# NeRdTheNed/deft4j

Measured on AMD Instinct MI355X. Metric: input MB/s on raw-deflate optimise (mode NONE), higher is better.
Workload: dtype u8

## Files before the change

deft4j_amd/csrc/d4g_fused.h:

```cpp
#pragma once
#include "d4g_ops.h"

#define D4F_MAXSLOTS 576
#define D4F_MAXOPS 640
#define D4F_MAXM 256
#define D4F_MAXC 96
#define D4F_MAXH 384
#define D4F_PASSN 1024
#define D4F_LEASTN 64
#define D4F_HDRN 256
#define D4F_SWEEP_K 8
#define D4F_CODE_FIXED 1
#define D4F_MAXROUNDS 16
#define D4F_HS_SLOTS 8
#define D4F_TREE_SLOTS 4

struct D4FCode {
    uint8_t lens[D4G_NLIT + D4G_NDIST];
    int32_t nLit, nDist, type, err;
    int32_t pad[12];
};
struct D4FPairs {
    uint16_t pairs[D4G_MAXPAIRS];
    int32_t nPairs, pad[3];
};
struct D4FHdr {
    uint8_t clLen[32];
    uint32_t flags[10];
    int32_t nCl, bits, base, pad;
    int32_t pad2[2];
};
struct D4FGlob {
    uint32_t* hist;
    D4FCode* code;
    D4FPairs* pairs;
    D4FHdr* hdr;
    int32_t* binBase;
};
#define D4F_GLOB_BYTES ((size_t)D4F_MAXM * D4G_HIST * 4 + (size_t)D4F_MAXC * sizeof(D4FCode) + (size_t)(D4F_MAXC + 1) * sizeof(D4FPairs) + \
                        (size_t)D4F_MAXH * sizeof(D4FHdr) + (size_t)D4F_MAXC * 64 * 4)

struct D4FParams {
    const D4GOp* ops[2];
    int32_t nOps[2];
    int32_t maxRounds;
    int32_t regWords;
    uint32_t caps;
    int32_t pad;
    D4GRoundResult* results;
    int32_t* roundInfo;
    long long* stats;
};
#define D4F_CL_MAXT 48
#define D4F_CL_SLOTS 96
#define D4F_CL_CHUNK (64 * D4F_NWR)
#define D4F_CL_SWEEP_WORDS 16
enum { D4F_CMD_SWEEP = 1, D4F_CMD_APPLY = 2, D4F_CMD_LEAST_WALK = 3, D4F_CMD_LEAST_EXPAND = 4 };
struct D4FClTask {
    int32_t m, code, prune, leaf, mNew, mode, rem, via;
    uint32_t full;
    int32_t pad0[3];
    int32_t cnt, saved;
    unsigned long long h1, h2;
    int32_t bin[3][32];
    int32_t delta[D4G_HIST];
    int32_t pad1[14];
};
static_assert(sizeof(D4FClTask) % 128 == 0, "tasks on cache lines of their own");
struct D4FClCmd {
    int32_t cmd, nItems, nTasks, nk, nChunks, pad0[3];
    int32_t codes[D4F_SWEEP_K];
    int32_t next, done, pad1[14];
    uint32_t neq[D4F_SWEEP_K];
    int32_t pad2[24];
    D4FClTask task[D4F_CL_MAXT];
};
struct D4FClArena {
    int32_t epoch;
    int32_t pad[31];
    D4FClCmd slot[D4F_CL_SLOTS];
};

#define D4F_CAPS(masks, codes, hdrs) ((uint32_t)(masks) | (uint32_t)(hdrs) << 10 | (uint32_t)(codes) << 20)
#define D4F_INFO_FALLBACK 0x10000
#define D4F_INFO_MORE 0x20000

struct D4FSlot { int16_t m, c, h; uint8_t valid, type; int32_t lazy; long long litlen; };
struct D4FPassE { uint32_t key; int32_t saved; int16_t mOut; uint8_t st, pad; };
struct D4FLeastE { uint32_t key; int32_t delta; int16_t mOut; uint8_t st, pad; };
struct D4FHdrE { uint32_t key; int16_t hOut; uint8_t st, pad; };

enum { D4F_Q_SWEEP = 0, D4F_Q_APPLY, D4F_Q_BINBASE, D4F_Q_LEAST, D4F_Q_TREE, D4F_Q_HDR, D4F_Q_HS, D4F_Q_FIXDOT, D4F_NQ };
#define D4F_QCAP_SWEEP D4F_MAXC
#define D4F_QCAP_APPLY 256
#define D4F_QCAP_BINBASE D4F_MAXC
#define D4F_QCAP_LEAST 64
#define D4F_QCAP_TREE 64
#define D4F_QCAP_HDR 256
#define D4F_QCAP_HS D4F_MAXC
#define D4F_QCAP_FIXDOT 4
#define D4F_QTOTAL (D4F_QCAP_SWEEP + D4F_QCAP_APPLY + D4F_QCAP_BINBASE + D4F_QCAP_LEAST + D4F_QCAP_TREE + D4F_QCAP_HDR + D4F_QCAP_HS + D4F_QCAP_FIXDOT)
D4G_DEV int d4f_qcap(int q) {
    return q == D4F_Q_SWEEP ? D4F_QCAP_SWEEP : q == D4F_Q_APPLY ? D4F_QCAP_APPLY : q == D4F_Q_BINBASE ? D4F_QCAP_BINBASE : q == D4F_Q_LEAST ? D4F_QCAP_LEAST
         : q == D4F_Q_TREE ? D4F_QCAP_TREE : q == D4F_Q_HDR ? D4F_QCAP_HDR : q == D4F_Q_HS ? D4F_QCAP_HS : D4F_QCAP_FIXDOT;
}
D4G_DEV int d4f_qoff(int q) {
    int o = 0;
    if (q > D4F_Q_SWEEP) o += D4F_QCAP_SWEEP;
    if (q > D4F_Q_APPLY) o += D4F_QCAP_APPLY;
    if (q > D4F_Q_BINBASE) o += D4F_QCAP_BINBASE;
    if (q > D4F_Q_LEAST) o += D4F_QCAP_LEAST;
    if (q > D4F_Q_TREE) o += D4F_QCAP_TREE;
    if (q > D4F_Q_HDR) o += D4F_QCAP_HDR;
    if (q > D4F_Q_HS) o += D4F_QCAP_HS;
    return o;
}
enum { D4F_H_OPT = 1, D4F_H_POST = 2, D4F_H_PRUNE = 3 };

typedef TreeMem<uint64_t, uint16_t, D4G_NLIT, 16, true> D4FLitTree;
typedef TreeMem<uint64_t, uint16_t, D4G_NDIST, 16, true> D4FDistTree;
struct D4FTreeScr {
    alignas(16) unsigned char tree[(D4FLitTree::bytes(1) + 15) & ~15];
    alignas(16) unsigned char treeD[(D4FDistTree::bytes(1) + 15) & ~15];
    uint32_t hist[D4G_HIST];
    alignas(16) uint8_t lens[D4G_NLIT + D4G_NDIST];
    uint16_t pairs[D4G_MAXPAIRS];
    uint8_t clLen[32];
    uint32_t clFreq[20];
    int32_t nLit, nDist, nCl, nPairs, hdrBits, err, m, pad;
    long long litlen;
};
struct D4FWaveScr {
    uint32_t hist[D4G_HIST];
    uint16_t lc[256];
    uint8_t cl[64];
    uint32_t queue[128];
    int32_t binSize[32], binFreq[32], binZ[32];
    int32_t delta[D4G_HIST];
    int32_t misc[16];
};
struct D4FHdrScr {
    uint16_t pairs[D4G_MAXPAIRS];
    uint8_t clLen[32];
    uint32_t clFreq[20];
    alignas(16) unsigned char tree[256];
    int32_t nCl, nPairs, bits, pad;
};
struct D4FSweepScr {
    uint16_t lc[D4F_SWEEP_K][256];
    uint8_t cl[D4F_SWEEP_K][64];
    uint32_t neq[D4F_SWEEP_K];
    unsigned long long stage[8][D4F_SWEEP_K][2][16];
};
struct D4FHsScr {
    D4GHdrLds H;
    alignas(16) uint8_t comb[D4G_NLIT + D4G_NDIST];
};
union D4FScratch {
    D4FTreeScr tree[D4F_TREE_SLOTS];
    D4FWaveScr wave[8];
    D4FSweepScr sweep;
    D4GLds levelLds;
};
static_assert(sizeof(D4FHdrScr) <= sizeof(D4FWaveScr), "header scratch overlays the wave scratch");

struct D4FLds {
    D4FSlot slot[D4F_MAXSLOTS];
    uint8_t slotReady[D4F_MAXSLOTS];
    uint8_t opStage[D4F_MAXOPS];
    uint16_t opReq[D4F_MAXOPS];
    long long treeLit[D4F_MAXM];
    uint8_t treeC[D4F_MAXM];
    alignas(4) uint8_t treeSt[D4F_MAXM];
    int32_t hdrBits[D4F_MAXH];
    unsigned long long maskH1[D4F_MAXM], maskH2[D4F_MAXM];
    int32_t maskPop[D4F_MAXM];
    uint32_t maskFull[D4F_MAXM];
    alignas(4) uint16_t maskHash[512];
    uint16_t maskStep[D4F_MAXM];
    uint16_t maskHH[D4F_MAXM];
    int32_t treeCand[2][D4F_QCAP_TREE];
    int16_t defHdr[D4F_MAXC];
    uint16_t qAll[D4F_QTOTAL];
    int32_t qn[D4F_NQ];
    int32_t nMask, nHdr, nDone, fallback, progress[2], fixdotSt, fixdotM, step, pad0;
    long long fixdotLit;
    long long red[32];
    int32_t misc[32];
    alignas(16) D4FLeastE least[D4F_LEASTN];
    D4FHdrE hdrReq[D4F_HDRN];
    D4FPassE pass[D4F_PASSN];
    D4FScratch scr;
    unsigned long long codeH[D4F_MAXC];
    alignas(4) uint8_t codeHash[256];
    alignas(4) uint8_t eState[D4F_MAXC];
    alignas(4) uint8_t eEq[D4F_MAXC];
    alignas(4) uint8_t bbState[D4F_MAXC];
    alignas(4) uint8_t hsState[D4F_MAXC];
    int32_t hsBits[D4F_MAXC];
    alignas(4) uint8_t hsLane[D4F_MAXC];
    int32_t nCode, capC;
    D4GCtx c;
    D4GBlock b;
    D4FGlob G;
    const D4GOp* ops;
    int32_t nOps, curType, rounds, info, improved, regWords;
    struct D4FClArena* cl;
    int32_t clEpoch, clDoneWg;
    int32_t which;
    int16_t capM, capH;
    long long curSize;
};

static_assert(sizeof(D4FLds) <= 80 * 1024, "two workgroups per CU: 80 KiB of LDS each");
static_assert(offsetof(D4FLds, codeH) - offsetof(D4FLds, least) >= D4F_HS_SLOTS * sizeof(D4FHsScr), "header-search scratch overlay");
__shared__ D4FLds d4fLds;
#define D4F_TASK __device__ __attribute__((noinline))
// ... 1140 lines not shown
        if (lane < 32) dst.clLen[lane] = H.clLen[lane];
        if (lane < 10) {
            uint32_t fl = 0;
            for (int j = 0; j < 32; j++) { const int i = lane * 32 + j; if (i < nPairs && (H.pairs[i] & D4G_PAIR_EXPANDED)) fl |= 1u << j; }
            dst.flags[lane] = fl;
        }
        if (lane == 0) { dst.nCl = H.nCl; dst.bits = H.bits; dst.base = src.base; F.hdrBits[hNew] = H.bits; }
    }
    d4g_wave_sync();
    if (lane == 0) { e.hOut = (int16_t)hNew; d4g_fence_block(); e.st = 2; }
}

D4F_TASK void d4f_tree_lit(int slotIdx, int m) {
    D4FLds& F = d4fLds;
    D4F_CTX;
    D4FTreeScr& T = F.scr.tree[slotIdx];
    const int lane = threadIdx.x & 63;
    for (int i = lane; i < D4G_NLIT; i += 64) T.hist[i] = G.hist[(size_t)m * D4G_HIST + i];
    for (int i = lane; i < D4G_NLIT / 4; i += 64) ((uint32_t*)T.lens)[i] = 0;
    d4g_wave_sync();
    int ml = 0;
    for (int i = lane; i < 286; i += 64) if (T.hist[i]) ml = i + 1 > ml ? i + 1 : ml;
    const int lastLit = wave_max_i32(ml);
    D4FLitTree tm;
    tm.carve(T.tree, 1);
    const int err = d4f_wave_tree<(D4G_NLIT + 63) / 64>(tm, lastLit, 15, [&](int i) { return T.hist[i]; }, [&](int v, int len) { T.lens[v] = (uint8_t)len; });
    if (lane == 0) { T.nLit = lastLit; T.err = err; T.m = m; }
    d4g_wave_sync();
}
D4F_TASK void d4f_tree_dist(int slotIdx, int m) {
    D4FLds& F = d4fLds;
    D4F_CTX;
    D4FTreeScr& T = F.scr.tree[slotIdx];
    const int lane = threadIdx.x & 63;
    if (lane < D4G_NDIST) { T.hist[D4G_NLIT + lane] = G.hist[(size_t)m * D4G_HIST + D4G_NLIT + lane]; T.lens[D4G_NLIT + lane] = 0; }
    d4g_wave_sync();
    int md = 0;
    if (lane < 30 && T.hist[D4G_NLIT + lane]) md = lane + 1;
    const int lastDist = wave_max_i32(md);
    const bool used = lane < lastDist && T.hist[D4G_NLIT + lane] != 0;
    const int nz = __popcll(d4g_ballot(used));
    int nDist, err = 0;
    if (lastDist == 0) nDist = 1;
    else if (nz <= 1) { nDist = lastDist; if (lane == 0) T.lens[D4G_NLIT + lastDist - 1] = 1; }
    else {
        D4FDistTree tm;
        tm.carve(T.treeD, 1);
        err = d4f_wave_tree<1>(tm, lastDist, 15, [&](int i) { return T.hist[D4G_NLIT + i]; }, [&](int v, int len) { T.lens[D4G_NLIT + v] = (uint8_t)len; });
        nDist = lastDist;
    }
    if (lane == 0) { T.nDist = nDist; T.pad = err; }
    d4g_wave_sync();
}
D4F_TASK void d4f_tree_header(int slotIdx) {
    D4FLds& F = d4fLds;
    D4FTreeScr& T = F.scr.tree[slotIdx];
    const int lane = threadIdx.x & 63;
    long long v = 0;
    for (int i = lane; i < D4G_HIST; i += 64) {
        const unsigned h = T.hist[i];
        if (h) {
            if (i < D4G_NLIT) v += (long long)h * (T.lens[i] + (i >= 257 ? d4g_lsym_ebits(i) : 0));
            else v += (long long)h * (T.lens[i] + d4g_dsym_ebits(i - D4G_NLIT));
        }
    }
    v = wave_sum_i64(v);
    int nPairs, nCl, bits;
    const int err = d4f_wave_default_header(T.lens, T.nLit, T.nDist, T.pairs, T.clFreq, T.clLen, T.tree, nPairs, nCl, bits);
    if (lane == 0) { T.nCl = nCl; T.nPairs = nPairs; T.hdrBits = bits; T.err |= err | T.pad; T.litlen = v; }
    d4g_wave_sync();
}
D4F_TASK void d4f_tree_publish(int slotIdx) {
    D4FLds& F = d4fLds;
    D4F_CTX;
    D4FTreeScr& T = F.scr.tree[slotIdx];
    const int lane = threadIdx.x & 63;
    unsigned long long h = 0;
    const uint32_t* lw = (const uint32_t*)T.lens;
    for (int i = lane; i < (D4G_NLIT + D4G_NDIST) / 4; i += 64) h += d4f_mix1(i, lw[i]);
    h = (unsigned long long)wave_sum_i64((long long)h) + (unsigned long long)T.nLit * 0x100000001b3ULL + ((unsigned long long)T.nDist << 48);
    if (h == 0) h = 1;
    int found = -1;
    uint32_t k = (uint32_t)(h >> 40) & 255u;
    for (int probe = 0; probe < 256; probe++, k = (k + 1) & 255u) {
        const int e = F.codeHash[k];
        if (e == 0) break;
        const int id = e - 1;
        if (F.codeH[id] == h) {
            const D4FCode& cd = G.code[id];
            int bad = 0;
            for (int i = lane; i < (D4G_NLIT + D4G_NDIST) / 4; i += 64) bad |= ((const uint32_t*)cd.lens)[i] != lw[i];
            if (lane == 0) bad |= cd.nLit != T.nLit || cd.nDist != T.nDist || cd.type != D4G_DYNAMIC;
            if (!d4g_ballot(bad)) { found = id; break; }
        }
    }
    int code = found;
    const int nCodeNow = __shfl(F.nCode, 0);
    if (code < 0) {
        code = nCodeNow;
        if (code >= F.capC) { if (lane == 0) F.fallback = 1; code = 0; }
        else {
            D4FCode& cd = G.code[code];
            for (int i = lane; i < (D4G_NLIT + D4G_NDIST) / 4; i += 64) ((uint32_t*)cd.lens)[i] = lw[i];
            if (lane == 0) {
                cd.nLit = T.nLit; cd.nDist = T.nDist; cd.type = D4G_DYNAMIC; cd.err = T.err;
                F.nCode = code + 1;
                F.codeH[code] = h;
                F.defHdr[code] = -1;
                F.eState[code] = 0; F.eEq[code] = 0; F.bbState[code] = 0; F.hsState[code] = 0;
                F.codeHash[k] = (uint8_t)(code + 1);
            }
        }
    }
    d4g_wave_sync();
    if (T.err && lane == 0) atomicAdd(c.errors, 1);
    const int defNow = __shfl((int)F.defHdr[code], 0);
    const int nHdrNow = __shfl(F.nHdr, 0);
    if (defNow < 0) {
        int hid = nHdrNow;
        if (hid >= F.capH) { if (lane == 0) F.fallback = 1; hid = 0; }
        else {
            D4FPairs& pb = G.pairs[1 + code];
            for (int i = lane; i < T.nPairs; i += 64) pb.pairs[i] = T.pairs[i];
            D4FHdr& hd = G.hdr[hid];
            if (lane < 32) hd.clLen[lane] = lane < 19 ? T.clLen[lane] : 0;
            if (lane < 10) hd.flags[lane] = 0;
            if (lane == 0) {
                pb.nPairs = T.nPairs;
                hd.nCl = T.nCl; hd.bits = T.hdrBits; hd.base = 1 + code;
                F.hdrBits[hid] = T.hdrBits;
                F.nHdr = hid + 1;
                F.defHdr[code] = (int16_t)hid;
            }
        }
    }
    d4g_wave_sync();
    if (lane == 0) { F.treeC[T.m] = (uint8_t)code; F.treeLit[T.m] = T.litlen; d4g_fence_block(); F.treeSt[T.m] = 2; }
    d4g_wave_sync();
}

D4F_TASK int d4f_hs_task(int slotIdx, int code) {
    D4FLds& F = d4fLds;
    D4F_CTX;
    D4FHsScr& X = ((D4FHsScr*)&F.least)[slotIdx];
    const int lane = threadIdx.x & 63;
    D4GHdrLds& H = X.H;
    uint8_t* comb = X.comb;
    const D4FCode& cd = G.code[code];
    const int nLit = cd.nLit, n = nLit + cd.nDist;
    for (int i = lane; i < (D4G_NLIT + D4G_NDIST) / 4; i += 64) ((uint32_t*)H.lens)[i] = ((const uint32_t*)cd.lens)[i];
    d4g_wave_sync();
    for (int i = lane; i < D4G_NLIT + D4G_NDIST; i += 64) comb[i] = i >= n ? 0 : i < nLit ? H.lens[i] : H.lens[D4G_NLIT + i - nLit];
    if (lane < 20) H.baseFreq[lane] = 0;
    d4g_wave_sync();
    {
        constexpr int NCH = (D4G_NLIT + D4G_NDIST) / 64;
        unsigned long long sm[NCH];
        int v[NCH];
#pragma unroll
        for (int ch = 0; ch < NCH; ch++) {
            int i = ch * 64 + lane;
            v[ch] = i < n ? (int)comb[i] : -1;
            int pv = (i > 0 && i < n) ? (int)comb[i - 1] : -2;
            sm[ch] = d4g_ballot(i < n && v[ch] != pv);
        }
        int ncx = 0;
#pragma unroll
        for (int ch = 0; ch < NCH; ch++) {
            int i = ch * 64 + lane;
            bool start = (sm[ch] >> lane) & 1;
            int run = 0;
            if (start) {
                int nx = -1;
                unsigned long long m = lane == 63 ? 0ULL : (sm[ch] >> (lane + 1));
                if (m) nx = i + __ffsll((long long)m);
#pragma unroll
                for (int c2 = ch + 1; c2 < NCH; c2++)
                    if (nx < 0 && sm[c2]) nx = c2 * 64 + __ffsll((long long)sm[c2]) - 1;
                if (nx < 0) nx = n;
                run = nx - i;
            }
            bool simple = start && (v[ch] != 0 ? run <= 3 : run <= 2);
            bool cx = start && !simple;
            if (simple) atomicAdd(&H.baseFreq[v[ch]], (unsigned)run);
            unsigned long long cm = d4g_ballot(cx);
// ... 379 lines not shown
    D4FGlob G;
    uint8_t* p = (uint8_t*)state_ptr(c, blk, 1);
    G.hist = (uint32_t*)p; p += (size_t)D4F_MAXM * D4G_HIST * 4;
    G.code = (D4FCode*)p; p += (size_t)D4F_MAXC * sizeof(D4FCode);
    G.pairs = (D4FPairs*)p; p += (size_t)(D4F_MAXC + 1) * sizeof(D4FPairs);
    G.hdr = (D4FHdr*)p; p += (size_t)D4F_MAXH * sizeof(D4FHdr);
    G.binBase = (int32_t*)p;
    return G;
}

__device__ __forceinline__ void d4f_assemble(const D4FGlob& G, D4GState* S, int mid, int cid, int hid, int type, long long litlen) {
    const D4FCode& cd = G.code[cid];
    __syncthreads();
    for (int i = threadIdx.x; i < (D4G_NLIT + D4G_NDIST) / 4; i += blockDim.x) ((uint32_t*)S->litLen)[i] = ((const uint32_t*)cd.lens)[i];
    for (int i = threadIdx.x; i < D4G_HIST; i += blockDim.x) S->hist[i] = G.hist[(size_t)mid * D4G_HIST + i];
    for (int i = threadIdx.x; i < 8; i += blockDim.x) ((uint32_t*)S->clLen)[i] = 0;
    if (type == D4G_DYNAMIC) {
        const D4FHdr& hd = G.hdr[hid];
        const D4FPairs& pb = G.pairs[hd.base];
        const int np = pb.nPairs;
        for (int i = threadIdx.x; i < np; i += blockDim.x) S->pairs[i] = (uint16_t)(pb.pairs[i] | (((hd.flags[i >> 5] >> (i & 31)) & 1u) ? D4G_PAIR_EXPANDED : 0u));
        __syncthreads();
        if (threadIdx.x < 32) S->clLen[threadIdx.x] = hd.clLen[threadIdx.x];
        if (threadIdx.x == 0) { S->nCl = hd.nCl; S->nPairs = np; S->hdrBits = hd.bits; S->nLit = cd.nLit; S->nDist = cd.nDist; }
    } else {
        if (threadIdx.x == 0) { S->nCl = 0; S->nPairs = 0; S->hdrBits = 0; S->nLit = 0; S->nDist = 0; }
    }
    __syncthreads();
    if (threadIdx.x == 0) {
        S->valid = 1; S->type = type; S->maskSlot = 0; S->flags = 0; S->pad0 = 0;
        S->litlenBits = litlen;
        S->sizeBits = litlen + S->hdrBits;
    }
    __syncthreads();
}

D4F_TASK bool d4f_round_setup(const D4GOp* ops0, const D4GOp* ops1, int nOps0, int nOps1) {
    D4FLds& F = d4fLds;
    D4F_CTX;
    const int lane = threadIdx.x & 63, wave = threadIdx.x >> 6;
    const D4GState* cur = state_ptr(c, c.active[d4fLds.which], 0);
    __syncthreads();
    const int curType = cur->type;
    const int prog = curType == D4G_FIXED ? 1 : 0;
    const int nOps = prog ? nOps1 : nOps0;
    for (int i = threadIdx.x; i < (int)(offsetof(D4FLds, scr) / 4); i += blockDim.x) ((uint32_t*)&F)[i] = 0;
    __syncthreads();
    if (threadIdx.x == 0) { F.ops = prog ? ops1 : ops0; F.nOps = nOps; F.curType = curType; F.curSize = cur->sizeBits; }
    if (nOps > D4F_MAXOPS || c.slotsPerBlock > D4F_MAXSLOTS) { __syncthreads(); return false; }
    if (F.nCode > D4F_MAXC - 32) {
        __syncthreads();
        for (int i = threadIdx.x; i < D4F_MAXC; i += blockDim.x) { F.eState[i] = 0; F.eEq[i] = 0; F.bbState[i] = 0; F.hsState[i] = 0; }
        for (int i = threadIdx.x; i < 256; i += blockDim.x) F.codeHash[i] = 0;
        if (threadIdx.x == 0) F.nCode = 2;
        __syncthreads();
    }
    for (int i = threadIdx.x; i < D4F_MAXC; i += blockDim.x) F.defHdr[i] = -1;
    D4FCode& c1 = G.code[D4F_CODE_FIXED];
    for (int i = threadIdx.x; i < D4G_NLIT + D4G_NDIST; i += blockDim.x)
        c1.lens[i] = (uint8_t)(i < 144 ? 8 : i < 256 ? 9 : i < 280 ? 7 : i < 286 ? 8 : i < D4G_NLIT ? 0 : i < D4G_NLIT + 30 ? 5 : 0);
    for (int i = threadIdx.x; i < D4G_HIST; i += blockDim.x) G.hist[i] = cur->hist[i];
    D4FPairs& p0 = G.pairs[0];
    D4FHdr& h0 = G.hdr[0];
    const int np = curType == D4G_DYNAMIC ? cur->nPairs : 0;
    for (int i = threadIdx.x; i < np; i += blockDim.x) p0.pairs[i] = (uint16_t)(cur->pairs[i] & ~D4G_PAIR_EXPANDED);
    if (threadIdx.x < 10) {
        uint32_t fl = 0;
        for (int j = 0; j < 32; j++) { const int i = threadIdx.x * 32 + j; if (i < np && (cur->pairs[i] & D4G_PAIR_EXPANDED)) fl |= 1u << j; }
        h0.flags[threadIdx.x] = fl;
    }
    if (threadIdx.x < 32) h0.clLen[threadIdx.x] = curType == D4G_DYNAMIC ? cur->clLen[threadIdx.x] : 0;
    int pc = 0;
    const uint64_t* m0 = d4f_mask(c, b, 0);
    for (int w = threadIdx.x; w < (int)b.maskWords; w += blockDim.x) pc += __popcll(m0[w]);
    const long long pop = wg_sum_i64(pc, F.red);
    {
        const uint64_t* bmask = c.binMask + b.binMask;
        const int nWords = (int)b.maskWords;
        unsigned nf = 0;
        if (nWords > 4096) nf = (1u << D4G_NBINS) - 1;
        else for (int i = threadIdx.x; i < D4G_NBINS * nWords; i += blockDim.x) {
            const int bin = i / nWords, w = i - bin * nWords;
            if (bmask[(long long)bin * nWords + w] & ~m0[w]) nf |= 1u << bin;
        }
        if (nf) atomicOr((unsigned*)&F.misc[1], nf);
        __syncthreads();
        if (threadIdx.x == 0) F.maskFull[0] = ~(unsigned)F.misc[1] & ((1u << D4G_NBINS) - 1);
    }
    if (wave == 0) {
        const uint32_t* cw = (const uint32_t*)cur->litLen;
        const uint32_t w0 = cw[lane], w1 = lane < 16 ? cw[64 + lane] : 0u;
        const int nLit0 = cur->nLit, nDist0 = cur->nDist;
        unsigned long long h = d4f_mix1(lane, w0) + (lane < 16 ? d4f_mix1(64 + lane, w1) : 0ull);
        h = (unsigned long long)wave_sum_i64((long long)h) + (unsigned long long)nLit0 * 0x100000001b3ULL + ((unsigned long long)nDist0 << 48) +
            (curType == D4G_DYNAMIC ? 0ull : 0x9e3779b97f4a7c15ULL);
        if (h == 0) h = 1;
        int found = -1;
        uint32_t k = (uint32_t)(h >> 40) & 255u;
        for (int probe = 0; probe < 256; probe++, k = (k + 1) & 255u) {
            const int e = F.codeHash[k];
            if (e == 0) break;
            const int id = e - 1;
            if (F.codeH[id] == h) {
                const D4FCode& cd = G.code[id];
                int bad = ((const uint32_t*)cd.lens)[lane] != w0;
                if (lane < 16) bad |= ((const uint32_t*)cd.lens)[64 + lane] != w1;
                if (lane == 0) bad |= cd.nLit != nLit0 || cd.nDist != nDist0 || cd.type != curType;
                if (!d4g_ballot(bad)) { found = id; break; }
            }
        }
        const int nCodeNow = __shfl(F.nCode, 0);
        int code = found;
        if (code < 0) {
            code = nCodeNow;
            D4FCode& cd = G.code[code];
            ((uint32_t*)cd.lens)[lane] = w0;
            if (lane < 16) ((uint32_t*)cd.lens)[64 + lane] = w1;
            if (lane == 0) {
                cd.nLit = nLit0; cd.nDist = nDist0; cd.type = curType; cd.err = 0;
                F.nCode = code + 1;
                F.codeH[code] = h;
                F.codeHash[k] = (uint8_t)(code + 1);
                F.eState[code] = 0; F.eEq[code] = 0; F.bbState[code] = 0; F.hsState[code] = 0;
            }
        }
        if (lane == 0) F.misc[2] = code;
    }
    if (wave == 1 || blockDim.x == 64) {
        const uint16_t hh = d4f_hist_hash(cur->hist);
        if (lane == 0) F.maskHH[0] = hh;
    }
    __syncthreads();
    if (threadIdx.x == 0) {
        c1.nLit = 0; c1.nDist = 0; c1.type = D4G_FIXED; c1.err = 0;
        p0.nPairs = np;
        h0.nCl = cur->nCl; h0.bits = (int32_t)cur->hdrBits; h0.base = 0;
        F.hdrBits[0] = curType == D4G_DYNAMIC ? (int32_t)cur->hdrBits : 0;
        F.nMask = 1; F.nHdr = 1; F.step = 1;
        F.maskPop[0] = (int)pop;
        D4FSlot s;
        s.m = 0; s.c = (int16_t)F.misc[2]; s.h = 0; s.valid = 1; s.type = (uint8_t)curType; s.lazy = 0; s.litlen = cur->litlenBits;
        F.slot[0] = s;
        F.slotReady[0] = 1;
    }
    __syncthreads();
    return true;
}

D4F_TASK bool d4f_select(long long best, D4GRoundResult* out) {
    D4FLds& F = d4fLds;
    D4F_CTX;
    const int wave = threadIdx.x >> 6;
    D4GState* cur = state_ptr(c, c.active[d4fLds.which], 0);
    const long long curSize = F.curSize;
    const long long bestSize = best >> D4G_KEY_SEQ_BITS;
    const int seq = (int)(best & ((1 << D4G_KEY_SEQ_BITS) - 1));
    const bool improved = best != D4G_KEY_NONE && bestSize < curSize;
    int newType = F.curType;
    __syncthreads();
    if (improved) {
        const int opId = seq >> 6, hl = seq & 63;
        const D4GOp op = F.ops[opId];
        const bool fromSrc = op.kind == OP_CAND || op.kind == OP_HDRSEARCH;
        const D4FSlot ws = F.slot[fromSrc ? op.src : op.dst];
        int mid = ws.m;
        __syncthreads();
        if (ws.lazy) {
            if (threadIdx.x == 0) {
                F.pass[0].key = 1u + ((uint32_t)ws.m | ((uint32_t)ws.c << 8));
                F.pass[0].st = 0;
            }
            __syncthreads();
// ... 22 lines not shown
            uint64_t* md = d4f_mask(c, b, 0);
            for (int w = threadIdx.x; w < (int)b.maskWords; w += blockDim.x) md[w] = ms[w];
        }
        __syncthreads();
        newType = S->type;
        for (int i = threadIdx.x; i < (int)(sizeof(D4GState) / 4); i += blockDim.x) ((uint32_t*)cur)[i] = ((const uint32_t*)S)[i];
        __syncthreads();
    }
    if (threadIdx.x == 0) {
        D4GRoundResult r;
        r.curSize = curSize;
        r.bestSize = improved ? bestSize : curSize;
        r.bestSeq = improved ? (seq >> 6) : -1;
        r.improved = improved ? 1 : 0;
        r.newType = newType;
        r.pad = 0;
        *out = r;
        F.improved = improved ? 1 : 0;
    }
    __syncthreads();
    return true;
}

__device__ __forceinline__ void d4f_block_init(const D4GCtx& cArg, const D4FParams& P, int which, D4FClArena* arena) {
    D4FLds& F = d4fLds;
    for (int i = threadIdx.x; i < D4F_MAXC; i += blockDim.x) { F.eState[i] = 0; F.eEq[i] = 0; F.bbState[i] = 0; F.hsState[i] = 0; }
    for (int i = threadIdx.x; i < 256; i += blockDim.x) F.codeHash[i] = 0;
    if (threadIdx.x == 0) {
        const int blk = cArg.active[which];
        F.nCode = 2;
        F.regWords = P.regWords < 64 * D4F_NWR ? P.regWords : 64 * D4F_NWR;
        const int capM = (int)(P.caps & 1023u), capH = (int)((P.caps >> 10) & 1023u), capC = (int)(P.caps >> 20);
        F.capM = (int16_t)(capM < D4F_MAXM ? capM : D4F_MAXM);
        F.capC = capC < D4F_MAXC ? capC : D4F_MAXC;
        F.capH = (int16_t)(capH < D4F_MAXH ? capH : D4F_MAXH);
        F.c = cArg;
        F.b = cArg.blocks[blk];
        F.G = d4f_glob(cArg, blk);
        F.cl = arena;
        F.clEpoch = 0;
        F.which = which;
    }
    __syncthreads();
}

__device__ __forceinline__ void d4f_block_rounds(const D4FParams& P) {
    D4FLds& F = d4fLds;
    const int which = F.which;
    const int lane = threadIdx.x & 63, wave = threadIdx.x >> 6, nw = blockDim.x >> 6;
    int rounds = 0, info = 0;
    const bool prof = P.stats != nullptr && threadIdx.x == 0;
    auto acc = [&](int k, long long v) { if (prof) atomicAdd((unsigned long long*)&P.stats[k], (unsigned long long)v); };
    const long long tKernel = prof ? clock64() : 0;
    for (;;) {
        long long tp = prof ? clock64() : 0;
        if (!d4f_round_setup(P.ops[0], P.ops[1], P.nOps[0], P.nOps[1])) { info |= D4F_INFO_FALLBACK; break; }
        if (prof) { acc(25, clock64() - tp); acc(27, 1); }
        const D4GOp* ops = F.ops;
        const int nOps = F.nOps;
        D4GOp myOp0, myOp1;
        memset(&myOp0, 0, sizeof(myOp0));
        memset(&myOp1, 0, sizeof(myOp1));
        if ((int)threadIdx.x < nOps) myOp0 = ops[threadIdx.x];
        if ((int)(threadIdx.x + blockDim.x) < nOps) myOp1 = ops[threadIdx.x + blockDim.x];
        long long bestKey = D4G_KEY_NONE;
        int guard = 0;
        int lastWhich = -1;
        auto may_move = [&](int kind, int stage) -> bool {
            if (stage == 0 || lastWhich < 0) return true;
            switch (kind) {
            case OP_HDRSEARCH: return lastWhich == D4F_Q_HS;
            case OP_POST: case OP_PRUNEHDR: return lastWhich == D4F_Q_HDR;
            case OP_OPT: return lastWhich == D4F_Q_APPLY || lastWhich == D4F_Q_HDR;
            case OP_RECODE: case OP_RECODE_FULL: return stage == 1 ? lastWhich == D4F_Q_APPLY : lastWhich == D4F_Q_TREE;
            case OP_LEAST: return lastWhich == D4F_Q_LEAST;
            case OP_TOFIXED_OPT: return stage == 1 ? lastWhich == D4F_Q_FIXDOT : lastWhich == D4F_Q_APPLY;
            default: return true;
            }
        };
        for (int iter = 0;; iter++) {
            bool prog2 = false;
            tp = prof ? clock64() : 0;
            for (int i = threadIdx.x, n = 0; i < nOps; i += blockDim.x, n++) {
                const int st = F.opStage[i];
                if (st == 255) continue;
                const D4GOp& o = n == 0 ? myOp0 : n == 1 ? myOp1 : ops[i];
                if (F.slotReady[o.src] && may_move(o.kind, st)) prog2 |= d4f_advance_op(o, i, &bestKey);
            }
            if (prog2) F.progress[iter & 1] = 1;
            __syncthreads();
            if (prof) { acc(24, clock64() - tp); acc(28, 1); }
            const int nDone = F.nDone, fb = F.fallback, progressed = F.progress[iter & 1];
            int which = -1;
            for (int q = 0; q < D4F_NQ; q++)
                if (q != D4F_Q_HS && F.qn[q] > 0) { which = q; break; }
            if (which < 0 && !progressed && F.qn[D4F_Q_HS] > 0) which = D4F_Q_HS;
            if (threadIdx.x == 0) { F.step++; F.progress[(iter + 1) & 1] = 0; }
            __syncthreads();
            if (fb) break;
            if (nDone >= nOps) break;
            lastWhich = which;
            if (which < 0) {
                if (!progressed && ++guard > 4) { if (threadIdx.x == 0) { atomicAdd(F.c.errors, 1); F.fallback = 1; } __syncthreads(); break; }
                continue;
            }
            guard = 0;
            const int nq = F.qn[which] < d4f_qcap(which) ? F.qn[which] : d4f_qcap(which);
            if (prof) { acc(which, nq); acc(8 + which, 1); tp = clock64(); }
            switch (which) {
            case D4F_Q_SWEEP: if (F.cl) d4f_cl_sweep(); else d4f_sweep(); break;
            case D4F_Q_APPLY:
                if (F.cl) { d4f_cl_apply_phase(nq); break; }
                for (int t = wave; t < nq; t += nw) d4f_apply_task(F.qAll[d4f_qoff(D4F_Q_APPLY) + t]);
                break;
            case D4F_Q_BINBASE: d4f_binbase(); break;
            case D4F_Q_LEAST:
                if (F.cl) { d4f_cl_least_phase(nq); break; }
                for (int t = wave; t < nq; t += nw) d4f_least_task(F.qAll[d4f_qoff(D4F_Q_LEAST) + t]);
                break;
            case D4F_Q_TREE: {
                uint16_t* Q = &F.qAll[d4f_qoff(D4F_Q_TREE)];
                const int nMaskNow = F.nMask;
                if ((int)threadIdx.x < nq) { F.treeCand[0][threadIdx.x] = 0x7fffffff; F.treeCand[1][threadIdx.x] = 0x7fffffff; }
                __syncthreads();
                for (int i = threadIdx.x; i < nq * nMaskNow; i += blockDim.x) {
                    const int t = i / nMaskNow, mp = i - t * nMaskNow, m = Q[t];
                    if (mp != m && F.treeSt[mp] == 2 && F.maskHH[mp] == F.maskHH[m]) atomicMin(&F.treeCand[0][t], mp);
                }
                for (int i = threadIdx.x; i < nq * nq; i += blockDim.x) {
                    const int t = i / nq, j = i - t * nq;
                    if (j < t && F.maskHH[Q[j]] == F.maskHH[Q[t]]) atomicMin(&F.treeCand[1][t], j);
                }
                __syncthreads();
                for (int t = wave; t < nq; t += nw) {
                    const int m = Q[t];
                    int from = F.treeCand[0][t] != 0x7fffffff ? F.treeCand[0][t] : F.treeCand[1][t] != 0x7fffffff ? (int)Q[F.treeCand[1][t]] : -1;
                    if (from >= 0) {
                        int diff = 0;
                        for (int i = lane; i < D4G_HIST; i += 64) diff |= F.G.hist[(size_t)m * D4G_HIST + i] != F.G.hist[(size_t)from * D4G_HIST + i];
                        if (d4g_ballot(diff)) from = -1;
                    }
                    d4g_wave_sync();
                    if (lane == 0) F.treeCand[0][t] = from;
                }
                __syncthreads();
                if (threadIdx.x == 0) {
                    int nu = 0, na = 0;
                    for (int t = 0; t < nq; t++) {
                        const int m = Q[t], from = F.treeCand[0][t];
                        if (from < 0) Q[nu++] = (uint16_t)m;
                        else F.treeCand[1][na++] = (m << 16) | from;
                    }
                    F.misc[3] = nu;
                }
                __syncthreads();
                const int nu = F.misc[3];
                if (prof) acc(38, nq - nu);
                const int nts = (nw >> 1) < D4F_TREE_SLOTS ? (nw >> 1) : D4F_TREE_SLOTS;
                const bool distWave = wave >= nts;
                const int ts = distWave ? wave - nts : wave;
                for (int t0 = 0; t0 < nu; t0 += nts) {
                    long long tq = prof ? clock64() : 0;
                    if (ts < nts && t0 + ts < nu) {
                        const int m = Q[t0 + ts];
                        if (distWave) d4f_tree_dist(ts, m); else d4f_tree_lit(ts, m);
                    }
                    if (prof) { acc(33, clock64() - tq); tq = clock64(); }
                    __syncthreads();
                    if (prof) { acc(34, clock64() - tq); tq = clock64(); }
                    if (ts < nts && t0 + ts < nu && !distWave) d4f_tree_header(ts);
                    __syncthreads();
                    if (prof) { acc(35, clock64() - tq); tq = clock64(); }
                    if (wave == 0)
                        for (int t = 0; t < nts && t0 + t < nu; t++) d4f_tree_publish(t);
                    __syncthreads();
                    if (prof) { acc(36, clock64() - tq); acc(37, 1); }
                }
                if (threadIdx.x == 0) {
                    for (int k = 0; k < nq - nu; k++) {
                        const int m = F.treeCand[1][k] >> 16, from = F.treeCand[1][k] & 0xffff;
                        F.treeC[m] = F.treeC[from]; F.treeLit[m] = F.treeLit[from];
                        d4g_fence_block();
                        F.treeSt[m] = 2;
                    }
                }
                break;
            }
            case D4F_Q_HDR:
                for (int t = wave; t < nq; t += nw) d4f_hdr_task(F.qAll[d4f_qoff(D4F_Q_HDR) + t]);
                break;
            case D4F_Q_HS: {
                const int nhs = nw < D4F_HS_SLOTS ? nw : D4F_HS_SLOTS;
                for (int t0 = 0; t0 < nq; t0 += nhs) {
                    if (wave < nhs && t0 + wave < nq) {
                        const int nfb = d4f_hs_task(wave, F.qAll[d4f_qoff(D4F_Q_HS) + t0 + wave]);
                        if (P.stats && lane == 0 && nfb) atomicAdd((unsigned long long*)&P.stats[62], (unsigned long long)nfb);
                    }
                    __syncthreads();
                }
                break;
            }
            case D4F_Q_FIXDOT: {
                const int m = F.qAll[d4f_qoff(D4F_Q_FIXDOT) + 0];
                long long v = 0;
                const uint8_t* ln = F.G.code[D4F_CODE_FIXED].lens;
                for (int i = threadIdx.x; i < D4G_HIST; i += blockDim.x) {
                    const unsigned h = F.G.hist[(size_t)m * D4G_HIST + i];
                    if (h) v += (long long)h * (ln[i] + (i < D4G_NLIT ? (i >= 257 ? d4g_lsym_ebits(i) : 0) : d4g_dsym_ebits(i - D4G_NLIT)));
                }
                v = wg_sum_i64(v, F.red);
                if (threadIdx.x == 0) { F.fixdotLit = v; F.fixdotSt = 2; }
                break;
            }
            default: break;
            }
            __syncthreads();
            if (prof) acc(16 + which, clock64() - tp);
            if (threadIdx.x == 0) F.qn[which] = 0;
            __syncthreads();
        }
        if (prof) { acc(30, F.nMask); acc(31, F.nCode); acc(32, F.nHdr); }
        if (F.fallback) { info |= D4F_INFO_FALLBACK; break; }
        long long best = wave_min_i64(bestKey);
        __syncthreads();
        if (lane == 0) F.red[wave] = best;
        __syncthreads();
        for (int i = 0; i < nw; i++) best = F.red[i] < best ? F.red[i] : best;
        __syncthreads();
        tp = prof ? clock64() : 0;
// ... 61 lines not shown
```

deft4j_amd/csrc/d4g_program.h:

```cpp
#pragma once
#include <algorithm>
#include <cstring>
#include <map>
#include <mutex>
#include <set>
#include <vector>

#include "d4g_knobs.h"

namespace d4g {

typedef long long i64;

struct Program {
    std::vector<D4GOp> ops;
    std::vector<int> opLevel;
    std::vector<int> slotLevel;
    int nSlots = 1, nMasks = 1, nLevels = 0;
    std::vector<std::vector<int>> stateLevels, hdrLevels;
    RtBuf<D4GOp> dOps;
    RtBuf<int32_t> dLists;
    std::vector<std::pair<size_t, int>> stateOff, hdrOff;
    int nRequested = 0;
    std::set<int> hsCodes;
// ... 237 lines not shown
                                        prune[k] = (uint8_t)pr;
                                        k++;
                                    }
                            } else {
                                flags[k] = (uint8_t)base;
                                prune[k] = (uint8_t)pr;
                                k++;
                            }
                        }
    if (k != 56) throw std::runtime_error("header flag table: expected 56 candidates");
}

struct Engine {
    Program progDyn, progFixed;
    RtBuf<uint8_t> dHdrTables;
    RtBuf<long long> dOpStats;
    RtBuf<uint32_t> dCrcTab;
    int slotsPerBlock = 0, masksPerBlock = 0, maxOps = 0;
    bool ready = false, built = false;
    void release() {
        if (!ready) return;
        progDyn.release(); progFixed.release();
        dHdrTables.reset(); dOpStats.reset(); dCrcTab.reset();
        ready = false;
    }
    void init() {
        static std::mutex initMu;
        std::lock_guard<std::mutex> lk(initMu);
        if (ready) return;
        if (!built) {
            progDyn.build(false);
            progFixed.build(true);
            built = true;
        }
        const int dbg = debug_program();
        if (dbg)
            fprintf(stderr, "program: %d ops requested, %zu emitted (%zu header searches over %zu distinct code-length sets), %d levels, %d slots, %d masks\n",
                    progDyn.nRequested, progDyn.ops.size(), (size_t)std::count_if(progDyn.ops.begin(), progDyn.ops.end(), [](const D4GOp& o) { return o.kind == OP_HDRSEARCH; }),
                    progDyn.hsCodes.size(), progDyn.nLevels, progDyn.nSlots, progDyn.nMasks);
        if (dbg >= 2)
            for (int l = 0; l < progDyn.nLevels; l++) {
                int kinds[16] = {0};
                for (int id : progDyn.stateLevels[l]) kinds[progDyn.ops[id].kind * 1 + 0]++;
                fprintf(stderr, "level %2d: OPT %d RECODE %d FULL %d LEAST %d POST %d PRUNEHDR %d TOFIXED %d CAND %d | hdr searches %zu\n", l, kinds[1], kinds[2],
                        kinds[3], kinds[4], kinds[5], kinds[6], kinds[7], kinds[8], progDyn.hdrLevels[l].size());
            }
        progDyn.upload();
        progFixed.upload();
        uint8_t tab[128];
        memset(tab, 0, sizeof(tab));
        build_hdr_tables(tab, tab + 64);
        dHdrTables.alloc(128);
        rt_h2d(dHdrTables, tab, 128);
        dOpStats.alloc_zero(64);
        {
            std::vector<uint32_t> t(1024 + 32);
            for (uint32_t i = 0; i < 256; i++) {
                uint32_t c = i;
                for (int k = 0; k < 8; k++) c = (c & 1) ? (c >> 1) ^ 0xedb88320u : c >> 1;
                t[i] = c;
            }
            for (int k = 1; k < 4; k++)
                for (uint32_t i = 0; i < 256; i++) t[k * 256 + i] = (t[(k - 1) * 256 + i] >> 8) ^ t[t[(k - 1) * 256 + i] & 0xff];
            auto mul = [](uint32_t a, uint32_t b) {
                uint32_t m = 1u << 31, p = 0;
                for (;;) {
                    if (a & m) { p ^= b; if ((a & (m - 1)) == 0) break; }
                    m >>= 1;
                    b = (b & 1) ? (b >> 1) ^ 0xedb88320u : b >> 1;
                }
                return p;
            };
            uint32_t p = 1u << 30;
            t[1024] = p;
            for (int k = 1; k < 32; k++) t[1024 + k] = p = mul(p, p);
            dCrcTab.alloc(t.size());
            rt_h2d(dCrcTab, t.data(), t.size() * 4);
        }
        rt_sync();
        slotsPerBlock = std::max(progDyn.nSlots, progFixed.nSlots);
        masksPerBlock = std::max(progDyn.nMasks, progFixed.nMasks);
        slotsPerBlock = std::max<int>(slotsPerBlock, 2 + (int)((D4F_GLOB_BYTES + sizeof(D4GState) - 1) / sizeof(D4GState)));
        masksPerBlock = std::max<int>(masksPerBlock, D4F_MAXM + 2 * D4F_MAXC);
        maxOps = (int)std::max(progDyn.ops.size(), progFixed.ops.size());
        if ((i64)maxOps * 64 >= (1LL << D4G_KEY_SEQ_BITS)) throw std::runtime_error("program too long for the key layout");
        ready = true;
    }
};
inline Engine& engine() {
    static Engine e[RT_MAX_CTX];
    return e[rt_ctx()];
}

}
```

deft4j_amd/csrc/libdeft4g.hip:

```cpp
#include <functional>
#include <mutex>
#include <thread>

#include "d4g_host.h"
#include "d4g_lz77_host.h"
#include "d4g_zopfli_host.h"
#include "d4g_host_find.h"

using namespace d4g;

struct d4g_batch {
    int ctx = 0;
    Batch impl;
    std::unique_ptr<LzFront> lz;
    std::unique_ptr<Batch> reopt;
    std::vector<int> reoptIndex;
    std::vector<char> graft;
    std::vector<int64_t> recompSaved;
    bool verified = false;
    std::vector<int32_t> verdict;
    std::vector<int64_t> firstMismatch;
    std::vector<std::vector<Batch::PBlock>> finalBlocks;
    const HStream& final_stream(size_t i, const Batch** owner) const {
        if (i < graft.size() && graft[i]) { *owner = reopt.get(); return reopt->streams[reoptIndex[i]]; }
// ... 1287 lines not shown
    if ((which != 0 && which != 1) || (cap && !out)) return fail(D4G_ERR_ARG, "bad argument");
    if (b->impl.ps[i].status != 0) return fail(D4G_ERR_ARG, "stream did not parse");
    const std::vector<Batch::PBlock>* list = &b->impl.ps[i].blocks;
    if (which == 1 && b->impl.dOut && stream_written(*b, i) && (b->lz == nullptr || b->impl.streams[i].saved > 0)) {
        if (!b->verified)
            if (int rc = d4g_batch_verify(b)) return rc;
        if (b->finalBlocks[i].empty()) return fail(D4G_ERR_RUNTIME, "the final stream does not parse");
        list = &b->finalBlocks[i];
    }
    i64 pos = 0;
    for (size_t k = 0; k < list->size(); k++) {
        const Batch::PBlock& pb = (*list)[k];
        pos += 3;
        i64 size = pb.sizeBits;
        if (pb.type == D4G_STORED) {
            const i64 c = pos % 8;
            size = (pb.uLen + 4) * 8 + (c == 0 ? 0 : 8 - c);
        }
        if (k < cap) out[k] = d4g_block_info{pb.type, pb.bfinal, pos - 3, size + 3, pb.type == D4G_DYNAMIC ? pb.hdrBits : 0, pb.nTok, pb.uLen};
        pos += size;
    }
    if (n_blocks) *n_blocks = list->size();
    return D4G_OK;
}

#ifdef D4G_HOSTSIM
long long d4g_test_pack_kinds(void) {
    long long bad = 0;
    for (int flags = 0; flags < 256; flags++)
        for (int v = 0; v <= 7; v += 7)
            for (int r = 1; r <= 420; r++) {
                int a[19 * 160] = {0}, b[19 * 160] = {0};
                d4g_pack_run(v, r, flags, [&](int sym, int run, int) { a[sym * 160 + run]++; });
                d4g_pack_kinds(v, r, flags, [&](int sym, int run, int, int cnt) { b[sym * 160 + run] += cnt; }, [&](int cnt) { b[v * 160] += cnt; });
                for (int i = 0; i < 19 * 160; i++) bad += a[i] != b[i];
            }
    return bad;
}
#endif

int d4g_debug_device_blocks(int64_t* live) {
    if (!live) return fail(D4G_ERR_ARG, "null argument");
    return api(nullptr, [&] {
        *live = (int64_t)rt_live_blocks();
        return D4G_OK;
    });
}

int d4g_debug_fused_stats(long long* out64) {
    return api(nullptr, [&] {
        engine().init();
        rt_sync_all();
        rt_d2h(out64, engine().dOpStats, 64 * 8);
        rt_memset(engine().dOpStats, 0, 64 * 8);
        rt_sync();
        return D4G_OK;
    });
}

#ifdef D4G_PROFILE_OPS
int d4g_debug_set_experiment(long long mode) {
    return api(nullptr, [&] {
        rt_h2d(engine().dOpStats + 63, &mode, 8);
        rt_sync();
        return D4G_OK;
    });
}
int d4g_debug_opstats(long long* out64) {
    return api(nullptr, [&] {
        rt_d2h(out64, engine().dOpStats, 64 * 8);
        (void)hipMemcpyFromSymbol(out64 + 56, HIP_SYMBOL(d4g_dbg_counters), 7 * 8);
        (void)hipMemcpyFromSymbol(out64 + 28, HIP_SYMBOL(d4g_dbg_hdr), 4 * 8);
        (void)hipMemcpyFromSymbol(out64 + 16, HIP_SYMBOL(d4g_dbg_tree), 3 * 8);
        (void)hipMemcpyFromSymbol(out64 + 34, HIP_SYMBOL(d4g_dbg_pass), 4 * 8);
        return D4G_OK;
    });
}
#endif

}
```

Baseline: 16170.

## Cache default header per code and defer header building to parallel waves

Tree building no longer computes the default code-length header inline for every candidate. Each code now caches its default header (CL lengths, count, bits), so a duplicate code reuses it instead of rebuilding. New codes are queued and their headers are built afterwards by up to eight waves in parallel. The hash probe moves onto the otherwise idle dist wave. The cost is more state per code, an extra pass with barriers, and added profiling counters.

New measurement: 16860 (median of 6 runs). 1.04x the previous value.

```diff
diff --git a/deft4j_amd/csrc/d4g_fused.h b/deft4j_amd/csrc/d4g_fused.h
--- a/deft4j_amd/csrc/d4g_fused.h
+++ b/deft4j_amd/csrc/d4g_fused.h
@@ -18,8 +18,11 @@
 struct D4FCode {
     uint8_t lens[D4G_NLIT + D4G_NDIST];
     int32_t nLit, nDist, type, err;
-    int32_t pad[12];
+    uint8_t defClLen[20];
+    int32_t defNCl, defBits, defStands;
+    int32_t pad[4];
 };
+static_assert(sizeof(D4FCode) == 384, "the carve-up of the block's state slots (D4F_GLOB_BYTES)");
 struct D4FPairs {
     uint16_t pairs[D4G_MAXPAIRS];
     int32_t nPairs, pad[3];
@@ -51,6 +54,7 @@
     int32_t* roundInfo;
     long long* stats;
 };
+#define D4F_NSTATS 80
 #define D4F_CL_MAXT 48
 #define D4F_CL_SLOTS 96
 #define D4F_CL_CHUNK (64 * D4F_NWR)
@@ -124,10 +128,8 @@
     alignas(16) unsigned char treeD[(D4FDistTree::bytes(1) + 15) & ~15];
     uint32_t hist[D4G_HIST];
     alignas(16) uint8_t lens[D4G_NLIT + D4G_NDIST];
-    uint16_t pairs[D4G_MAXPAIRS];
-    uint8_t clLen[32];
-    uint32_t clFreq[20];
-    int32_t nLit, nDist, nCl, nPairs, hdrBits, err, m, pad;
+    int32_t nLit, nDist, err, m, pad, found;
+    unsigned long long codeH;
     long long litlen;
 };
 struct D4FWaveScr {
@@ -146,6 +148,13 @@
     alignas(16) unsigned char tree[256];
     int32_t nCl, nPairs, bits, pad;
 };
+struct D4FDefScr {
+    alignas(16) uint8_t lens[D4G_NLIT + D4G_NDIST];
+    uint16_t pairs[D4G_MAXPAIRS];
+    uint8_t clLen[32];
+    uint32_t clFreq[20];
+    alignas(16) unsigned char tree[256];
+};
 struct D4FSweepScr {
     uint16_t lc[D4F_SWEEP_K][256];
     uint8_t cl[D4F_SWEEP_K][64];
@@ -163,6 +172,7 @@
     D4GLds levelLds;
 };
 static_assert(sizeof(D4FHdrScr) <= sizeof(D4FWaveScr), "header scratch overlays the wave scratch");
+static_assert(sizeof(D4FDefScr) <= sizeof(D4FWaveScr), "default-header scratch overlays the wave scratch");
 
 struct D4FLds {
     D4FSlot slot[D4F_MAXSLOTS];
@@ -1409,7 +1419,7 @@
     if (lane == 0) { T.nDist = nDist; T.pad = err; }
     d4g_wave_sync();
 }
-D4F_TASK void d4f_tree_header(int slotIdx) {
+D4F_TASK void d4f_tree_bits(int slotIdx) {
     D4FLds& F = d4fLds;
     D4FTreeScr& T = F.scr.tree[slotIdx];
     const int lane = threadIdx.x & 63;
@@ -1422,23 +1432,15 @@
         }
     }
     v = wave_sum_i64(v);
-    int nPairs, nCl, bits;
-    const int err = d4f_wave_default_header(T.lens, T.nLit, T.nDist, T.pairs, T.clFreq, T.clLen, T.tree, nPairs, nCl, bits);
-    if (lane == 0) { T.nCl = nCl; T.nPairs = nPairs; T.hdrBits = bits; T.err |= err | T.pad; T.litlen = v; }
-    d4g_wave_sync();
-}
-D4F_TASK void d4f_tree_publish(int slotIdx) {
-    D4FLds& F = d4fLds;
-    D4F_CTX;
-    D4FTreeScr& T = F.scr.tree[slotIdx];
+    if (lane == 0) { T.err |= T.pad; T.litlen = v; }
+    d4g_wave_sync();
+}
+D4G_DEV int d4f_code_probe(const D4FTreeScr& T, unsigned long long h, uint32_t& k) {
+    D4FLds& F = d4fLds;
+    const D4FGlob& G = F.G;
     const int lane = threadIdx.x & 63;
-    unsigned long long h = 0;
     const uint32_t* lw = (const uint32_t*)T.lens;
-    for (int i = lane; i < (D4G_NLIT + D4G_NDIST) / 4; i += 64) h += d4f_mix1(i, lw[i]);
-    h = (unsigned long long)wave_sum_i64((long long)h) + (unsigned long long)T.nLit * 0x100000001b3ULL + ((unsigned long long)T.nDist << 48);
-    if (h == 0) h = 1;
-    int found = -1;
-    uint32_t k = (uint32_t)(h >> 40) & 255u;
+    k = (uint32_t)(h >> 40) & 255u;
     for (int probe = 0; probe < 256; probe++, k = (k + 1) & 255u) {
         const int e = F.codeHash[k];
         if (e == 0) break;
@@ -1448,19 +1450,81 @@
             int bad = 0;
             for (int i = lane; i < (D4G_NLIT + D4G_NDIST) / 4; i += 64) bad |= ((const uint32_t*)cd.lens)[i] != lw[i];
             if (lane == 0) bad |= cd.nLit != T.nLit || cd.nDist != T.nDist || cd.type != D4G_DYNAMIC;
-            if (!d4g_ballot(bad)) { found = id; break; }
-        }
-    }
+            if (!d4g_ballot(bad)) return id;
+        }
+    }
+    return -1;
+}
+D4F_TASK void d4f_tree_probe(int slotIdx) {
+    D4FLds& F = d4fLds;
+    D4FTreeScr& T = F.scr.tree[slotIdx];
+    const int lane = threadIdx.x & 63;
+    unsigned long long h = 0;
+    const uint32_t* lw = (const uint32_t*)T.lens;
+    for (int i = lane; i < (D4G_NLIT + D4G_NDIST) / 4; i += 64) h += d4f_mix1(i, lw[i]);
+    h = (unsigned long long)wave_sum_i64((long long)h) + (unsigned long long)T.nLit * 0x100000001b3ULL + ((unsigned long long)T.nDist << 48);
+    if (h == 0) h = 1;
+    uint32_t k;
+    const int found = d4f_code_probe(T, h, k);
+    if (lane == 0) { T.codeH = h; T.found = found; }
+    d4g_wave_sync();
+}
+D4F_TASK void d4f_def_header(int waveSlot, int entry, long long* stats) {
+    D4FLds& F = d4fLds;
+    D4F_CTX;
+    D4FDefScr& X = *(D4FDefScr*)&F.scr.wave[waveSlot];
+    const int lane = threadIdx.x & 63;
+    const long long t0 = stats ? clock64() : 0;
+    const int code = entry >> 16, hid = entry & 0xffff;
+    D4FCode& cd = G.code[code];
+    for (int i = lane; i < (D4G_NLIT + D4G_NDIST) / 4; i += 64) ((uint32_t*)X.lens)[i] = ((const uint32_t*)cd.lens)[i];
+    d4g_wave_sync();
+    int nPairs, nCl, bits;
+    const int err = d4f_wave_default_header(X.lens, cd.nLit, cd.nDist, X.pairs, X.clFreq, X.clLen, X.tree, nPairs, nCl, bits);
+    D4FPairs& pb = G.pairs[1 + code];
+    for (int i = lane; i < nPairs; i += 64) pb.pairs[i] = X.pairs[i];
+    D4FHdr& hd = G.hdr[hid];
+    if (lane < 32) hd.clLen[lane] = lane < 19 ? X.clLen[lane] : 0;
+    if (lane < 20) cd.defClLen[lane] = lane < 19 ? X.clLen[lane] : 0;
+    if (lane < 10) hd.flags[lane] = 0;
+    if (lane == 0) {
+        if (err) { cd.err |= err; atomicAdd(c.errors, 1); }
+        pb.nPairs = nPairs;
+        hd.nCl = nCl; hd.bits = bits; hd.base = 1 + code;
+        F.hdrBits[hid] = bits;
+        cd.defNCl = nCl; cd.defBits = bits; cd.defStands = 1;
+        if (stats) {
+            atomicAdd((unsigned long long*)&stats[64], 1ull);
+            atomicAdd((unsigned long long*)&stats[65], (unsigned long long)(clock64() - t0));
+        }
+    }
+    d4g_wave_sync();
+}
+D4F_TASK void d4f_tree_publish(int slotIdx, long long* stats) {
+    D4FLds& F = d4fLds;
+    D4F_CTX;
+    D4FTreeScr& T = F.scr.tree[slotIdx];
+    const int lane = threadIdx.x & 63;
+    const uint32_t* lw = (const uint32_t*)T.lens;
+    const unsigned long long h = T.codeH;
+    int found = T.found;
+    uint32_t k = 0;
+    if (found < 0) {
+        found = d4f_code_probe(T, h, k);
+        if (stats && threadIdx.x == 0 && found >= 0) atomicAdd((unsigned long long*)&stats[71], 1ull);
+    }
+    if (stats && threadIdx.x == 0 && found >= 0) atomicAdd((unsigned long long*)&stats[70], 1ull);
     int code = found;
+    bool refused = false;
     const int nCodeNow = __shfl(F.nCode, 0);
     if (code < 0) {
         code = nCodeNow;
-        if (code >= F.capC) { if (lane == 0) F.fallback = 1; code = 0; }
+        if (code >= F.capC) { if (lane == 0) F.fallback = 1; code = 0; refused = true; }
         else {
             D4FCode& cd = G.code[code];
             for (int i = lane; i < (D4G_NLIT + D4G_NDIST) / 4; i += 64) ((uint32_t*)cd.lens)[i] = lw[i];
             if (lane == 0) {
-                cd.nLit = T.nLit; cd.nDist = T.nDist; cd.type = D4G_DYNAMIC; cd.err = T.err;
+                cd.nLit = T.nLit; cd.nDist = T.nDist; cd.type = D4G_DYNAMIC; cd.err = T.err; cd.defStands = 0;
                 F.nCode = code + 1;
                 F.codeH[code] = h;
                 F.defHdr[code] = -1;
@@ -1475,19 +1539,32 @@
     const int nHdrNow = __shfl(F.nHdr, 0);
     if (defNow < 0) {
         int hid = nHdrNow;
-        if (hid >= F.capH) { if (lane == 0) F.fallback = 1; hid = 0; }
-        else {
-            D4FPairs& pb = G.pairs[1 + code];
-            for (int i = lane; i < T.nPairs; i += 64) pb.pairs[i] = T.pairs[i];
-            D4FHdr& hd = G.hdr[hid];
-            if (lane < 32) hd.clLen[lane] = lane < 19 ? T.clLen[lane] : 0;
-            if (lane < 10) hd.flags[lane] = 0;
+        if (hid >= F.capH) {
+            if (lane == 0) F.fallback = 1;
+            hid = 0;
+            if (stats && threadIdx.x == 0) atomicAdd((unsigned long long*)&stats[72], 1ull);
+        } else {
+            const long long t0 = stats ? clock64() : 0;
+            const D4FCode& cd = G.code[code];
+            const int stands = found >= 0 ? __shfl(cd.defStands, 0) : 0;
+            if (stands) {
+                D4FHdr& hd = G.hdr[hid];
+                if (lane < 32) hd.clLen[lane] = lane < 19 ? cd.defClLen[lane] : 0;
+                if (lane < 10) hd.flags[lane] = 0;
+                if (lane == 0) {
+                    const int bits = cd.defBits;
+                    hd.nCl = cd.defNCl; hd.bits = bits; hd.base = 1 + code;
+                    F.hdrBits[hid] = bits;
+                }
+            }
             if (lane == 0) {
-                pb.nPairs = T.nPairs;
-                hd.nCl = T.nCl; hd.bits = T.hdrBits; hd.base = 1 + code;
-                F.hdrBits[hid] = T.hdrBits;
+                if (!stands && !refused) F.treeCand[0][F.misc[4]++] = (code << 16) | hid;
                 F.nHdr = hid + 1;
                 F.defHdr[code] = (int16_t)hid;
+                if (stats && stands && threadIdx.x == 0) {
+                    atomicAdd((unsigned long long*)&stats[66], 1ull);
+                    atomicAdd((unsigned long long*)&stats[67], (unsigned long long)(clock64() - t0));
+                }
             }
         }
     }
@@ -1973,6 +2050,7 @@
         __syncthreads();
         for (int i = threadIdx.x; i < D4F_MAXC; i += blockDim.x) { F.eState[i] = 0; F.eEq[i] = 0; F.bbState[i] = 0; F.hsState[i] = 0; }
         for (int i = threadIdx.x; i < 256; i += blockDim.x) F.codeHash[i] = 0;
+        for (int i = threadIdx.x; i < D4F_MAXC; i += blockDim.x) G.code[i].defStands = 0;
         if (threadIdx.x == 0) F.nCode = 2;
         __syncthreads();
     }
@@ -2038,7 +2116,7 @@
             ((uint32_t*)cd.lens)[lane] = w0;
             if (lane < 16) ((uint32_t*)cd.lens)[64 + lane] = w1;
             if (lane == 0) {
-                cd.nLit = nLit0; cd.nDist = nDist0; cd.type = curType; cd.err = 0;
+                cd.nLit = nLit0; cd.nDist = nDist0; cd.type = curType; cd.err = 0; cd.defStands = 0;
                 F.nCode = code + 1;
                 F.codeH[code] = h;
                 F.codeHash[k] = (uint8_t)(code + 1);
@@ -2167,6 +2245,8 @@
     const bool prof = P.stats != nullptr && threadIdx.x == 0;
     auto acc = [&](int k, long long v) { if (prof) atomicAdd((unsigned long long*)&P.stats[k], (unsigned long long)v); };
     const long long tKernel = prof ? clock64() : 0;
+    for (int i = threadIdx.x; i < D4F_MAXC; i += blockDim.x) F.G.code[i].defStands = 0;
+    __syncthreads();
     for (;;) {
         long long tp = prof ? clock64() : 0;
         if (!d4f_round_setup(P.ops[0], P.ops[1], P.nOps[0], P.nOps[1])) { info |= D4F_INFO_FALLBACK; break; }
@@ -2267,6 +2347,7 @@
                         else F.treeCand[1][na++] = (m << 16) | from;
                     }
                     F.misc[3] = nu;
+                    F.misc[4] = 0;
                 }
                 __syncthreads();
                 const int nu = F.misc[3];
@@ -2283,13 +2364,25 @@
                     if (prof) { acc(33, clock64() - tq); tq = clock64(); }
                     __syncthreads();
                     if (prof) { acc(34, clock64() - tq); tq = clock64(); }
-                    if (ts < nts && t0 + ts < nu && !distWave) d4f_tree_header(ts);
+                    if (ts < nts && t0 + ts < nu) {
+                        if (distWave) d4f_tree_probe(ts); else d4f_tree_bits(ts);
+                    }
                     __syncthreads();
                     if (prof) { acc(35, clock64() - tq); tq = clock64(); }
                     if (wave == 0)
-                        for (int t = 0; t < nts && t0 + t < nu; t++) d4f_tree_publish(t);
+                        for (int t = 0; t < nts && t0 + t < nu; t++) d4f_tree_publish(t, P.stats);
                     __syncthreads();
                     if (prof) { acc(36, clock64() - tq); acc(37, 1); }
+                }
+                const int nDef = F.misc[4];
+                if (nDef > 0) {
+                    const long long tq = prof ? clock64() : 0;
+                    const int nhw = nw < 8 ? nw : 8;
+                    for (int d0 = 0; d0 < nDef; d0 += nhw) {
+                        if (wave < nhw && d0 + wave < nDef) d4f_def_header(wave, F.treeCand[0][d0 + wave], P.stats);
+                        __syncthreads();
+                    }
+                    if (prof) { acc(68, 1); acc(69, clock64() - tq); }
                 }
                 if (threadIdx.x == 0) {
                     for (int k = 0; k < nq - nu; k++) {
diff --git a/deft4j_amd/csrc/d4g_program.h b/deft4j_amd/csrc/d4g_program.h
--- a/deft4j_amd/csrc/d4g_program.h
+++ b/deft4j_amd/csrc/d4g_program.h
@@ -313,7 +313,7 @@
         build_hdr_tables(tab, tab + 64);
         dHdrTables.alloc(128);
         rt_h2d(dHdrTables, tab, 128);
-        dOpStats.alloc_zero(64);
+        dOpStats.alloc_zero(D4F_NSTATS);
         {
             std::vector<uint32_t> t(1024 + 32);
             for (uint32_t i = 0; i < 256; i++) {
diff --git a/deft4j_amd/csrc/libdeft4g.hip b/deft4j_amd/csrc/libdeft4g.hip
--- a/deft4j_amd/csrc/libdeft4g.hip
+++ b/deft4j_amd/csrc/libdeft4g.hip
@@ -1363,7 +1363,17 @@
         engine().init();
         rt_sync_all();
         rt_d2h(out64, engine().dOpStats, 64 * 8);
-        rt_memset(engine().dOpStats, 0, 64 * 8);
+        rt_memset(engine().dOpStats, 0, D4F_NSTATS * 8);
+        rt_sync();
+        return D4G_OK;
+    });
+}
+int d4g_debug_fused_stats_all(long long* out80) {
+    return api(nullptr, [&] {
+        engine().init();
+        rt_sync_all();
+        rt_d2h(out80, engine().dOpStats, D4F_NSTATS * 8);
+        rt_memset(engine().dOpStats, 0, D4F_NSTATS * 8);
         rt_sync();
         return D4G_OK;
     });
```
